# byronknoll/gmix

Measured on AMD Instinct MI355X. Metric: mixer bits/sec (synthetic 256-input mixer streams, forward+update), higher is better.
Workload: dtype f32; 1 GPU; configs[1]: synthetic 256-input 1-layer mixer (1 mixer, 2^16-row gate table), random logits, forward+update; n_inputs=256, mixers=1/0/0, streams_per_gpu=4096, total_bits=5465178112, parallelism=streams sharded over 1 GPU(s), no collective on the data path

## Files before the change

gmix_amd/csrc/gmx_capi.cpp:

```cpp
#include <hip/hip_runtime.h>
#include <math.h>
#include <stddef.h>
#include <stdio.h>
#include <stdlib.h>
#include <string.h>
#include <time.h>

#include <algorithm>
#include <atomic>
#include <map>
#include <new>
#include <string>
#include <vector>

#include "../../include/gmxmix.h"
#include "../../include/gmxmix_lstm_group.h"
#include "../../include/gmxmix_decoder.h"
#include "gmx_buildhash.h"
#include "gmx_internal.h"
#include "gmx_mailbox.h"
#include "gmx_batch_rows.h"
#include "gmx_ckpt.h"
#include "gmx_ckpt_stage.h"
#include "gmx_ind_ckpt.h"
// ... 291 lines not shown
    void *dst = up ? *col.dev : *col.host, *src = up ? *col.host : *col.dev;
    const GmxRowCopy r = gmx_row_copy(c->S, c->max_rows, n, col.row_bytes);
    if (r.height)
      HIPCHK(hipMemcpy2DAsync(dst, r.pitch, src, r.pitch, r.width, r.height, kind, st));
    else
      HIPCHK(hipMemcpyAsync(dst, src, r.bytes, kind, st));
  }
  for (const GmxBatchCol& col : c->cols) {
    if (col.dir != dir || !col.per_stream) continue;
    void *dst = up ? *col.dev : *col.host, *src = up ? *col.host : *col.dev;
    HIPCHK(hipMemcpyAsync(dst, src, gmx_col_host_bytes(col, c->S, c->max_rows), kind, st));
  }
  return up ? xfer_end_upload(c->x, main, st) : xfer_end_download(c->x, st);
}
static int batch_core_wait(GmxBatchCore* c) {
  if (!c || !c->bank) return GMX_ERR_INVALID;
  HIPCHK(hipSetDevice(c->bank->device));
  return xfer_wait(c->x);
}


static constexpr int kStageSlots = 4;
struct GmxCountList {
  uint64_t* dev[kStageSlots] = {};
  uint64_t* host[kStageSlots] = {};
  hipEvent_t done[kStageSlots] = {};
  bool busy[kStageSlots] = {};
  size_t cap = 0;
  unsigned seq = 0;
};
static void count_list_free(GmxCountList& c) {
  for (int k = 0; k < kStageSlots; ++k) {
    if (c.dev[k]) (void)hipFree(c.dev[k]);
    if (c.host[k]) (void)hipHostFree(c.host[k]);
    if (c.done[k]) (void)hipEventDestroy(c.done[k]);
  }
  c = GmxCountList();
}
static int count_list_stage(GmxCountList& c, const uint64_t* counts, int n, hipStream_t st, const uint64_t** dev_out) {
  const int k = (int)(c.seq++ % (unsigned)kStageSlots);
  if (c.busy[k]) {
    HIPCHK(hipEventSynchronize(c.done[k]));
    c.busy[k] = false;
  }
  if ((size_t)n > c.cap) {
    for (int j = 0; j < kStageSlots; ++j) {
      if (c.busy[j]) {
        HIPCHK(hipEventSynchronize(c.done[j]));
        c.busy[j] = false;
      }
      if (c.dev[j]) (void)hipFree(c.dev[j]);
      if (c.host[j]) (void)hipHostFree(c.host[j]);
      c.dev[j] = nullptr;
      c.host[j] = nullptr;
    }
    c.cap = 0;
    const size_t cap = (size_t)n + 64;
    for (int j = 0; j < kStageSlots; ++j) {
      HIPCHK(hipMalloc((void**)&c.dev[j], cap * sizeof(uint64_t)));
      HIPCHK(hipHostMalloc((void**)&c.host[j], cap * sizeof(uint64_t), hipHostMallocDefault));
      if (!c.done[j]) HIPCHK(hipEventCreateWithFlags(&c.done[j], hipEventDisableTiming));
    }
    c.cap = cap;
  }
  memcpy(c.host[k], counts, (size_t)n * sizeof(uint64_t));
  HIPCHK(hipMemcpyAsync(c.dev[k], c.host[k], (size_t)n * sizeof(uint64_t), hipMemcpyHostToDevice, st));
  *dev_out = c.dev[k];
  return GMX_OK;
}
static int count_list_used(GmxCountList& c, hipStream_t st) {
  const int k = (int)((c.seq - 1u) % (unsigned)kStageSlots);
  HIPCHK(hipEventRecord(c.done[k], st));
  c.busy[k] = true;
  return GMX_OK;
}

struct gmx_group {
  int device = 0;
  int S = 0;
  GmxTopoDev topo;
  GmxTopoDev* topo_dev = nullptr;
  uint8_t* banks = nullptr;
  float* latch_out = nullptr;
  hipStream_t stream = nullptr;
  hipEvent_t ev0 = nullptr, ev1 = nullptr;
  unsigned lds_bytes = 0;
  std::vector<uint64_t> steps;
  std::vector<uint8_t> fwd_done;
  struct DecaySlot {
    float* dev = nullptr;
    uint32_t* idx_dev = nullptr;
    float* host = nullptr;
    uint32_t* idx_host = nullptr;
    size_t cap = 0;
    size_t idx_cap = 0;
    hipEvent_t done = nullptr;
    hipEvent_t ready = nullptr;
    bool busy = false;
    uint64_t* st_dev = nullptr;
    uint64_t* st_host = nullptr;
    uint32_t* amb_dev = nullptr;
    uint32_t* amb_host = nullptr;
    float* patch_host = nullptr;
    size_t st_cap = 0;
  } decay[kStageSlots];
  GmxCountList counts;
  hipStream_t copy_stream = nullptr;
  hipStream_t up_stream = nullptr, down_stream = nullptr;
  unsigned run_seq = 0;
  hipEvent_t tm0 = nullptr, tm1 = nullptr;
  gmx_batch* one = nullptr;
  GmxBatchBank bb;
  std::vector<struct GmxSession*> sessions;
  std::vector<struct gmx_lockstep*> locksteps;
  bool banks_in_use_by_dead_kernel = false;
  bool use_sessions = true;
  bool mailbox_on_device = true;
  bool force_general = false;
  bool stock_exact = false;
  int stock_staged = -1;
  bool decay_on_host = false;
  bool stock_pairs = false;
  bool register_rows = false;
  int single_variant = 0;
  struct GmxCkptState* ckpt = nullptr;
};

struct gmx_batch : GmxBatchCore {
  gmx_group* g = nullptr;
  uint64_t& max_bits = max_rows;
  unsigned flags = 0;
  float* d_pred = nullptr;
  uint32_t* d_mask = nullptr;
  uint32_t* d_ctx = nullptr;
  uint8_t* d_bits = nullptr;
  float* d_p = nullptr;
  float* d_out = nullptr;
  float* d_last = nullptr;
  uint64_t* d_rng = nullptr;
  uint64_t* d_tcount = nullptr;
  float* d_pstate = nullptr;
  uint32_t* d_cstate = nullptr;
  float* h_pred = nullptr;
  uint32_t* h_mask = nullptr;
  uint32_t* h_ctx = nullptr;
  uint8_t* h_bits = nullptr;
  float* h_p = nullptr;
  float* h_out = nullptr;
  float* h_last = nullptr;
};

struct gmx_lockstep {
  gmx_group* g = nullptr;
  gmx_batch* b = nullptr;
  float* dec_host = nullptr;
  uint8_t* bits_host = nullptr;
  float* dec_dev = nullptr;
  uint32_t* idx_dev = nullptr;
  hipGraph_t g_predict = nullptr, g_learn = nullptr, g_step = nullptr;
  hipGraphExec_t x_predict = nullptr, x_learn = nullptr, x_step = nullptr;
  bool predicted = false;
  bool persistent = false, ps_running = false, ps_dead = false, ps_counted = false;
  hipStream_t ps_stream = nullptr;
  GmxLsDoor* door = nullptr;
  uint32_t* done = nullptr;
  uint32_t* blk_seen = nullptr;
// ... 125 lines not shown
      x.rs_off = x.w_off + (uint64_t)at * 4u;
      x.rs_pitch = x.stride * 4u;
    } else {
      x.rs_off = off;
      x.rs_pitch = 8u;
      off += (uint64_t)x.table_size * 8u;
      off = round_up64(off, 128);
    }
  }
  o->scal_off = off;
  off += (uint64_t)o->m * 24u;
  o->bank_bytes = round_up64(off, 256);
  uint32_t l = 0;
  o->lds_in0 = l;
  o->in0_sz = round_up((uint32_t)o->n_pad + (uint32_t)o->l0 + 4u, 4);
  l += 2 * o->in0_sz;
  o->lds_o1 = l;
  l += round_up((uint32_t)(o->l1 ? o->l1 : 1), 4);
  o->lds_skip = l;
  l += GMX_MAX_SKIP;
  o->lds_misc = l;
  l += 256;
  for (int grp = 0; grp < 2; ++grp) {
    const int lo = grp == 0 ? 0 : o->l0, hi = grp == 0 ? o->l0 : o->m;
    if (lo >= hi) continue;
    uint32_t dmax = 0;
    for (int j = lo; j < hi; ++j) dmax = std::max(dmax, o->mx[j].stride);
    const uint32_t D = dmax + 4;
    const uint32_t S = round_up((uint32_t)(hi - lo) * D, 64);
    for (int j = lo; j < hi; ++j) {
      o->mx[j].lds_off = l + (uint32_t)(j - lo) * D;
      o->mx[j].pitch = S;
    }
    l += 2 * S;
  }
  o->lds_total = l;
  if ((uint64_t)o->lds_total * 4u > 160u * 1024u) return GMX_ERR_INVALID;
  return GMX_OK;
}

static void batch_free(gmx_batch* b);
static int batch_alloc(gmx_batch** out, gmx_group* g, int S, uint64_t max_bits, unsigned flags);
static int batch_note_device_use(gmx_batch* b);

extern "C" int gmx_group_create(gmx_group** out, const gmx_topology* topo, int n_streams, int device) {
  if (!out || n_streams < 1) return GMX_ERR_INVALID;
  *out = nullptr;
  GmxTopoDev td;
  int rc = build_topology(topo, &td);
  if (rc) return rc;
  int ndev = 0;
  if (hipGetDeviceCount(&ndev) != hipSuccess || ndev <= 0) {
    (void)hipGetLastError();
    return GMX_ERR_NO_DEVICE;
  }
  if (device < 0 || device >= ndev) return GMX_ERR_INVALID;
  HIPCHK(hipSetDevice(device));
  gmx_group* g = new (std::nothrow) gmx_group();
  if (!g) return GMX_ERR_NOMEM;
  g->device = device;
  batch_bank_init(g->bb, g, device, &g->stream, &g->up_stream, &g->down_stream);
  g->S = n_streams;
  g->topo = td;
  g->lds_bytes = td.lds_total * 4u;
  g->steps.assign(n_streams, 0);
  g->fwd_done.assign(n_streams, 0);
#define GCHK(call)                                 \
  do {                                             \
    hipError_t e_ = (call);                        \
    if (e_ != hipSuccess) {                        \
      int r_ = hip_fail(e_, #call);                \
      gmx_group_destroy(g);                        \
      return e_ == hipErrorOutOfMemory ? GMX_ERR_NOMEM : r_; \
    }                                              \
  } while (0)
  GCHK(bank_stream_create(&g->stream, 0));
  GCHK(hipEventCreate(&g->ev0));
  GCHK(hipEventCreate(&g->ev1));
  GCHK(hipMalloc((void**)&g->topo_dev, sizeof(GmxTopoDev)));
  GCHK(hipMemcpy(g->topo_dev, &g->topo, sizeof(GmxTopoDev), hipMemcpyHostToDevice));
  GCHK(hipMalloc((void**)&g->banks, (size_t)n_streams * td.bank_bytes));
  GCHK(hipMalloc((void**)&g->latch_out, (size_t)n_streams * td.m * sizeof(float)));
  GCHK(hipMemsetAsync(g->latch_out, 0, (size_t)n_streams * td.m * sizeof(float), g->stream));
  if (g->lds_bytes > 48u * 1024u) GCHK(gmx_bank_kernel_set_lds(g->lds_bytes));
#undef GCHK
  rc = gmx_group_reset(g);
  if (rc) {
    gmx_group_destroy(g);
    return rc;
  }
  *out = g;
  return GMX_OK;
}

extern "C" void gmx_group_destroy(gmx_group* g) {
  if (!g) return;
  (void)hipSetDevice(g->device);
  sessions_free(g);
  if (g->stream) (void)hipStreamSynchronize(g->stream);
  if (g->one) {
    batch_free(g->one);
    g->one = nullptr;
  }
  for (gmx_lockstep* ls : g->locksteps) ls->g = nullptr;
  g->locksteps.clear();
  batch_bank_detach_all(g->bb);
  if (!g->banks_in_use_by_dead_kernel) {
    if (g->banks) (void)hipFree(g->banks);
    if (g->latch_out) (void)hipFree(g->latch_out);
    if (g->topo_dev) (void)hipFree(g->topo_dev);
  }
  for (auto& d : g->decay) {
    if (d.st_dev) (void)hipFree(d.st_dev);
    if (d.st_host) (void)hipHostFree(d.st_host);
    if (d.amb_dev) (void)hipFree(d.amb_dev);
    if (d.amb_host) (void)hipHostFree(d.amb_host);
    if (d.patch_host) (void)hipHostFree(d.patch_host);
    if (d.dev) (void)hipFree(d.dev);
    if (d.idx_dev) (void)hipFree(d.idx_dev);
    if (d.host) (void)hipHostFree(d.host);
    if (d.idx_host) (void)hipHostFree(d.idx_host);
    if (d.done) (void)hipEventDestroy(d.done);
    if (d.ready) (void)hipEventDestroy(d.ready);
  }
  count_list_free(g->counts);
  ckpt_free(g);
  if (g->copy_stream) (void)hipStreamDestroy(g->copy_stream);
  if (g->up_stream) {
    (void)hipStreamSynchronize(g->up_stream);
    (void)hipStreamDestroy(g->up_stream);
  }
  if (g->down_stream) {
    (void)hipStreamSynchronize(g->down_stream);
    (void)hipStreamDestroy(g->down_stream);
  }
  if (g->tm0) (void)hipEventDestroy(g->tm0);
  if (g->tm1) (void)hipEventDestroy(g->tm1);
  if (g->ev0) (void)hipEventDestroy(g->ev0);
  if (g->ev1) (void)hipEventDestroy(g->ev1);
  if (g->stream) (void)hipStreamDestroy(g->stream);
  delete g;
}

extern "C" int gmx_group_n_streams(const gmx_group* g) { return g ? g->S : GMX_ERR_INVALID; }
extern "C" int gmx_group_n_mixers(const gmx_group* g) { return g ? g->topo.m : GMX_ERR_INVALID; }
extern "C" int gmx_group_n_inputs(const gmx_group* g) { return g ? g->topo.n : GMX_ERR_INVALID; }
extern "C" uint64_t gmx_group_bank_bytes(const gmx_group* g) { return g ? g->topo.bank_bytes : 0; }

extern "C" int gmx_group_reset(gmx_group* g) {
  if (!g) return GMX_ERR_INVALID;
  HIPCHK(hipSetDevice(g->device));
  int rc = sessions_close(g, false);
  if (rc) return rc;
  HIPCHK(hipMemsetAsync(g->banks, 0, (size_t)g->S * g->topo.bank_bytes, g->stream));
  HIPCHK(gmx_launch_init_scal(g->banks, g->topo.bank_bytes, g->topo.scal_off, g->topo.m, g->S,
                              g->stream));
  HIPCHK(hipStreamSynchronize(g->stream));
  std::fill(g->steps.begin(), g->steps.end(), 0);
  std::fill(g->fwd_done.begin(), g->fwd_done.end(), 0);
  for (gmx_lockstep* ls : g->locksteps) ls->predicted = false;
  return GMX_OK;
}

extern "C" int gmx_group_sync(gmx_group* g) {
  if (!g) return GMX_ERR_INVALID;
  HIPCHK(hipSetDevice(g->device));
  int rc = sessions_close(g, true);
  if (rc) return rc;
  HIPCHK(hipStreamSynchronize(g->stream));
  return GMX_OK;
}

extern "C" int gmx_group_timer_start(gmx_group* g) {
  if (!g) return GMX_ERR_INVALID;
  HIPCHK(hipSetDevice(g->device));
  if (!g->tm0) {
    HIPCHK(hipEventCreate(&g->tm0));
    HIPCHK(hipEventCreate(&g->tm1));
  }
  HIPCHK(hipEventRecord(g->tm0, g->stream));
  return GMX_OK;
}

extern "C" int gmx_group_timer_stop(gmx_group* g, float* ms) {
  if (!g || !ms || !g->tm0) return GMX_ERR_INVALID;
  HIPCHK(hipSetDevice(g->device));
  HIPCHK(hipEventRecord(g->tm1, g->stream));
  HIPCHK(hipEventSynchronize(g->tm1));
  HIPCHK(hipEventElapsedTime(ms, g->tm0, g->tm1));
  return GMX_OK;
}

// ... 99 lines not shown
      }
      if (!e.done) {
        HIPCHK(hipEventCreateWithFlags(&e.done, hipEventDisableTiming));
        HIPCHK(hipEventCreateWithFlags(&e.ready, hipEventDisableTiming));
      }
    }
  }
  if (!g->copy_stream) HIPCHK(sibling_stream_create(&g->copy_stream, g->stream));
  bool on_device = false;
  if (learn && uniq.size() > 1 && uniq.size() * T >= kDecayDeviceMin && uniq.size() * T < (1ull << 32) &&
      !g->decay_on_host) {
    const int rcd = decay_table_on_device(g, d, uniq, T);
    if (rcd != GMX_OK && rcd != GMX_ERR_STATE) return rcd;
    on_device = rcd == GMX_OK;
  }
  if (!on_device) {
    for (auto& kv : uniq) {
      float* tab = d.host + (size_t)kv.second * T;
      if (learn)
        for (uint64_t t = 0; t < T; ++t) tab[t] = decay_base(kv.first + t);
      else
        for (uint64_t t = 0; t < T; ++t) tab[t] = 0.f;
    }
    HIPCHK(hipMemcpyAsync(d.dev, d.host, uniq.size() * T * sizeof(float), hipMemcpyHostToDevice, g->copy_stream));
  }
  memcpy(d.idx_host, idx.data(), ns * sizeof(uint32_t));
  HIPCHK(hipMemcpyAsync(d.idx_dev, d.idx_host, ns * sizeof(uint32_t), hipMemcpyHostToDevice, g->copy_stream));
  HIPCHK(hipEventRecord(d.ready, g->copy_stream));
  HIPCHK(hipStreamWaitEvent(g->stream, d.ready, 0));
  return GMX_OK;
}

static bool topo_register_rows_eligible(const GmxTopoDev& t) {
  return t.has_final && t.l0 >= 1 && t.l0 <= 24 && t.l1 >= 1 && t.l1 <= 8 && t.m == t.l0 + t.l1 + 1 &&
         t.n_skip == 1 && gmx_pair_kernel_half(t.n) != 0;
}

enum GmxKernelKind : int { GMX_K_SINGLE, GMX_K_WIDE, GMX_K_STOCK, GMX_K_BANK, GMX_K_PAIR };
static GmxKernelKind kernel_for(const gmx_group* g, unsigned mode) {
  if (g->register_rows && (mode & GMX_MODE_PREDICT) && !(mode & GMX_MODE_LATCH) && !g->force_general &&
      topo_register_rows_eligible(g->topo))
    return GMX_K_PAIR;
  const bool single = g->topo.m == 1 && g->topo.n <= 256 && (mode & GMX_MODE_PREDICT) &&
                      !(mode & GMX_MODE_LATCH) && !g->force_general;
  const bool stock = g->topo.n == 90 && g->topo.l0 == 24 && g->topo.l1 == 8 && g->topo.n_skip == 1 &&
                     g->topo.has_final && g->topo.mx[23].stride == 128 && !g->force_general;
  const bool wide = g->topo.l0 == 24 && g->topo.l1 == 8 && g->topo.n_skip == 1 && g->topo.has_final &&
                    ((g->topo.n == 256 && g->topo.mx[23].stride == 288) ||
                     (g->topo.n == 90 && g->topo.mx[23].stride == 128 && g->stock_pairs && !g->stock_exact)) &&
                    (mode & GMX_MODE_PREDICT) && !(mode & GMX_MODE_LATCH) && !g->force_general;
  return single ? GMX_K_SINGLE : wide ? GMX_K_WIDE : stock ? GMX_K_STOCK : GMX_K_BANK;
}

static int launch_run(gmx_group* g, gmx_batch* b, int s0, int rec0, int ns, uint64_t T,
                      unsigned mode, float* kernel_ms, const uint64_t* n_list = nullptr) {
  if (T == 0) return GMX_OK;
  for (gmx_lockstep* ls : g->locksteps) ls->predicted = false;
  gmx_group::DecaySlot* dec = nullptr;
  int rc = prepare_decay(g, s0, ns, T, (mode & GMX_MODE_LEARN) ? 1 : 0, &dec);
  if (rc) return rc;
  GmxRunArgs a;
  memset(&a, 0, sizeof a);
  a.banks = g->banks;
  a.pred = b->d_pred;
  a.mask = (b->flags & GMX_BATCH_MASK) ? b->d_mask : nullptr;
  a.ctx = b->d_ctx;
  a.bits = b->d_bits;
  a.decay = dec->dev;
  a.decay_idx = dec->idx_dev;
  a.p_out = b->d_p;
  a.out_all = (b->flags & GMX_BATCH_OUTPUTS) ? b->d_out : nullptr;
  a.out_last = (b->flags & GMX_BATCH_LAST_OUTPUTS) ? b->d_last : nullptr;
  a.latch_out = g->latch_out;
  a.rec_stride = b->max_bits;
  a.T = T;
  if (n_list) {
    int rcl = count_list_stage(g->counts, n_list, ns, g->stream, &a.T_list);
    if (rcl) return rcl;
  }
  a.mode = mode | (g->stock_exact ? GMX_MODE_EXACT : 0u);
  a.stream_base = s0;
  a.rec_base = rec0;
  a.n_streams = ns;
  {
    int rcx = xfer_before_run(b->x, g->stream);
    if (rcx) return rcx;
  }
  if (kernel_ms) HIPCHK(hipEventRecord(g->ev0, g->stream));
  const GmxKernelKind kind = kernel_for(g, mode);
  const bool single = kind == GMX_K_SINGLE, wide = kind == GMX_K_WIDE, stock = kind == GMX_K_STOCK;
  if (a.out_last && (single || wide)) return GMX_ERR_INVALID;
  if (kind == GMX_K_PAIR)
    HIPCHK(gmx_launch_pair_kernel(g->topo_dev, &a, ns, a.mask != nullptr, g->topo.n, g->topo.l0, g->topo.l1, g->stream));
  else if (single)
    HIPCHK(gmx_launch_single_kernel(g->topo_dev, &a, g->topo.n, g->single_variant, g->stream));
  else if (wide)
    HIPCHK(gmx_launch_wide_kernel(g->topo_dev, &a, ns, a.mask != nullptr, g->topo.n, g->stream));
  else if (stock)
    HIPCHK(gmx_launch_stock_kernel(g->topo_dev, &a, ns, GMX_STK_LDS_BYTES(g->topo.lds_misc),
                                   a.mask != nullptr, g->stock_staged, topo_tables_pow2(g->topo), g->stream));
  else
    HIPCHK(gmx_launch_bank_kernel(g->topo_dev, &a, ns, g->lds_bytes, a.mask != nullptr, g->topo.l0,
                                  g->topo.l1, g->topo.n_skip, g->topo.has_final,
                                  g->topo.mx[g->topo.l0 - 1].stride, g->stream));
  HIPCHK(hipEventRecord(dec->done, g->stream));
  dec->busy = true;
  if (n_list) {
    int rcl = count_list_used(g->counts, g->stream);
    if (rcl) return rcl;
  }
  {
    int rcn = batch_note_device_use(b);
    if (rcn) return rcn;
  }
  if (kernel_ms) {
    HIPCHK(hipEventRecord(g->ev1, g->stream));
    HIPCHK(hipEventSynchronize(g->ev1));
    HIPCHK(hipEventElapsedTime(kernel_ms, g->ev0, g->ev1));
  }
  if (mode & GMX_MODE_LEARN)
    for (int i = 0; i < ns; ++i) g->steps[s0 + i] += n_list ? n_list[i] : T;
  return GMX_OK;
}

static void batch_free(gmx_batch* b) {
  if (!b) return;
  batch_core_free(*b);
  delete b;
}

static int batch_alloc(gmx_batch** out, gmx_group* g, int S, uint64_t max_bits, unsigned flags) {
  if (!out || !g || max_bits == 0) return GMX_ERR_INVALID;
  *out = nullptr;
  gmx_batch* b = new (std::nothrow) gmx_batch();
  if (!b) return GMX_ERR_NOMEM;
  b->back = (void**)&b->g;
  b->flags = flags;
  gmx_mixer_batch_cols(b->cols, b, g->topo.n_pad, g->topo.m, g->topo.mask_words, flags);
  int rc = batch_core_alloc(*b, &g->bb, S, max_bits, false);
  if (rc) {
    batch_free(b);
    return rc;
  }
  *out = b;
  return GMX_OK;
}

extern "C" int gmx_batch_create(gmx_batch** out, gmx_group* g, uint64_t max_bits, unsigned flags) {
  if (!g) return GMX_ERR_INVALID;
  if (flags & GMX_BATCH_LAST_OUTPUTS) {
    const GmxKernelKind kind = kernel_for(g, GMX_MODE_PREDICT | GMX_MODE_LEARN);
    if ((kind == GMX_K_SINGLE || kind == GMX_K_WIDE) && !topo_register_rows_eligible(g->topo)) return GMX_ERR_INVALID;
  }
  int rc = batch_alloc(out, g, g->S, max_bits, flags);
  if (rc) return rc;
  return xfer_streams_ready(g->stream, &g->up_stream, &g->down_stream);
}

extern "C" void gmx_batch_destroy(gmx_batch* b) { batch_free(b); }
extern "C" int gmx_batch_n_pad(const gmx_batch* b) { return (b && b->g) ? b->g->topo.n_pad : GMX_ERR_INVALID; }
extern "C" int gmx_batch_mask_words(const gmx_batch* b) { return (b && b->g) ? b->g->topo.mask_words : GMX_ERR_INVALID; }
extern "C" uint64_t gmx_batch_max_bits(const gmx_batch* b) { return b ? b->max_bits : 0; }

extern "C" float* gmx_batch_predictions(gmx_batch* b) { return b ? (float*)batch_core_host(*b, &b->h_pred) : nullptr; }
extern "C" uint32_t* gmx_batch_active_mask(gmx_batch* b) {
  return b ? (uint32_t*)batch_core_host(*b, &b->h_mask) : nullptr;
// ... 937 lines not shown
```

gmix_amd/csrc/gmx_internal.h:

```cpp
#ifndef GMX_INTERNAL_H_
#define GMX_INTERNAL_H_

#include <stdint.h>

#define GMX_MAX_MIXERS 64
#define GMX_MAX_SKIP 8
#define GMX_MAX_INPUTS 2048

#define GMX_MODE_PREDICT 1u
#define GMX_MODE_LEARN 2u
#define GMX_MODE_LATCH 4u
#define GMX_MODE_EXACT 8u

struct GmxMixerDev {
  uint32_t table_size;
  uint32_t weight_size;
  uint32_t stride;
  uint32_t lds_off;
  uint32_t pitch;
  int32_t layer;
  int32_t out_index;
  float lr;
  uint64_t w_off;
  uint64_t rs_off;
  uint32_t rs_pitch;
  uint32_t rs_folded;
};

#define GMX_RS_PTR(bank, mx, row) \
  ((uint64_t*)((uint8_t*)(bank) + (mx).rs_off + (uint64_t)(row) * (mx).rs_pitch))

struct GmxTopoDev {
  int32_t n, n_pad, n_skip, m, l0, l1, has_final, mask_words;
  int32_t skip_idx[GMX_MAX_SKIP];
  uint32_t lds_in0;
  uint32_t in0_sz;
  uint32_t lds_o1;
  uint32_t lds_skip;
  uint32_t lds_misc;
  uint32_t lds_total;
  uint64_t scal_off;
  uint64_t bank_bytes;
  GmxMixerDev mx[GMX_MAX_MIXERS];
};

struct GmxRunArgs {
  uint8_t* banks;
  const float* pred;
  const uint32_t* mask;
  const uint32_t* ctx;
  const uint8_t* bits;
  const float* decay;
  const uint32_t* decay_idx;
  float* p_out;
  float* out_all;
  float* out_last;
  float* latch_out;
  uint64_t rec_stride;
  uint64_t T;
  const uint64_t* T_list;
  uint32_t mode;
  int32_t stream_base;
  int32_t rec_base;
  int32_t n_streams;
};

#define GMX_STK_LDS_BYTES(lds_misc) (((lds_misc) + 256u) * 4u + 2u * 33u * 528u)

#define GMX_MB_FORWARD 1u
#define GMX_MB_LEARN0 2u
#define GMX_MB_LEARN1 3u
#define GMX_MB_STOP 4u
#define GMX_MB_LEARN0_FWD 5u
#define GMX_MB_LEARN1_FWD 6u
#define GMX_MB_STOP_KEEP 7u
#define GMX_MB_CMD_MASK 7u
#define GMX_MB_SLOT_SHIFT 3
#define GMX_MB_SEQ_SHIFT 4
#define GMX_MB_RUNNING 0u
#define GMX_MB_EXIT_IDLE 1u
#define GMX_MB_EXIT_STOP 2u
struct GmxMbPayload {
  uint32_t dec_bits;
  uint32_t pad0[3];
  uint32_t mask[4];
  uint32_t ctx[36];
  uint32_t pad1[4];
  float pred[96];
};
struct GmxMbCmd {
  uint32_t cmd_seq;
  uint32_t pad0[15];
  GmxMbPayload slot[2];
};
struct GmxMbReply {
  uint32_t done_seq;
  uint32_t state;
  float p;
  uint32_t pad[13];
  float outs[48];
};

struct GmxLsDoor {
  uint32_t cmd_seq;
  uint32_t pad[15];
};
struct GmxLsArgs {
  uint8_t* banks;
  GmxLsDoor* door;
  uint32_t* done;
  const float* pred;
  const uint32_t* mask;
  const uint32_t* ctx;
  const uint8_t* bits;
  const float* dec;
  float* p;
  float* outs;
  uint32_t* blk_seen;
  uint32_t* blk_replay;
  uint32_t* relay;
  float* live;
  uint64_t idle_ticks;
  int32_t n_streams, exact;
};
#define GMX_LS_LIVE_FLOATS 160

struct GmxStkStepArgs {
  uint8_t* banks;
  const uint8_t* what;
  const uint8_t* bits;
  const float* dec;
  const float* pred_old;
  const uint32_t* mask_old;
  const uint32_t* ctx_old;
  const float* pred_new;
  const uint32_t* mask_new;
  const uint32_t* ctx_new;
  float* p_out;
  float* out_all;
  float* latch;
  const uint32_t* seq;
  uint32_t* stamp;
  int32_t n_streams, exact;
};

#define GMX_STEP_UP_MAX 12
struct GmxStepUpload {
  const uint8_t* src;
// ... 182 lines not shown
```

gmix_amd/csrc/gmx_single.hip:

```cpp
#include <hip/hip_runtime.h>
#include <stdint.h>

#include "gmx_internal.h"
#include "gmx_math.h"

typedef float gmx_f4 __attribute__((ext_vector_type(4)));

template <int OFF>
__device__ __forceinline__ void gmx_ld16(gmx_f4& d, const float* p) {
  asm volatile("global_load_dwordx4 %0, %1, off offset:%2 nt" : "=v"(d) : "v"(p), "n"(OFF) : "memory");
}
__device__ __forceinline__ void gmx_ld8(uint64_t& d, const uint64_t* p) {
  asm volatile("global_load_dwordx2 %0, %1, off" : "=v"(d) : "v"(p) : "memory");
}
__device__ __forceinline__ void gmx_ld4(uint32_t& d, const void* p) {
  asm volatile("global_load_dword %0, %1, off" : "=v"(d) : "v"(p) : "memory");
}
__device__ __forceinline__ void gmx_ld1(uint32_t& d, const uint8_t* p) {
  asm volatile("global_load_ubyte %0, %1, off" : "=v"(d) : "v"(p) : "memory");
}
template <int OFF>
__device__ __forceinline__ void gmx_st16(float* p, const gmx_f4& v) {
  asm volatile("global_store_dwordx4 %0, %1, off offset:%2 nt" : : "v"(p), "v"(v), "n"(OFF) : "memory");
}
__device__ __forceinline__ void gmx_st8(uint64_t* p, uint64_t v) {
  asm volatile("global_store_dwordx2 %0, %1, off" : : "v"(p), "v"(v) : "memory");
}
__device__ __forceinline__ void gmx_st4(float* p, float v) {
  asm volatile("global_store_dword %0, %1, off" : : "v"(p), "v"(v) : "memory");
}

template <int K>
struct GmxSlot {
  gmx_f4 w[K];
  gmx_f4 x[K];
  uint32_t mk[K];
  uint64_t rs;
  uint32_t row;
  uint32_t bit;
  uint32_t dec;
};

template <int N>
__device__ __forceinline__ void gmx_wait_slot(GmxSlot<1>& a) {
  asm volatile("s_waitcnt vmcnt(%c5)"
               : "+v"(a.w[0]), "+v"(a.x[0]), "+v"(a.rs), "+v"(a.bit), "+v"(a.dec)
               : "n"(N));
}
template <int N>
__device__ __forceinline__ void gmx_wait_slot(GmxSlot<2>& a) {
  asm volatile("s_waitcnt vmcnt(%c7)"
               : "+v"(a.w[0]), "+v"(a.w[1]), "+v"(a.x[0]), "+v"(a.x[1]), "+v"(a.rs), "+v"(a.bit),
                 "+v"(a.dec)
               : "n"(N));
}
template <int N>
__device__ __forceinline__ void gmx_wait_slot(GmxSlot<4>& a) {
  asm volatile("s_waitcnt vmcnt(%c11)"
               : "+v"(a.w[0]), "+v"(a.w[1]), "+v"(a.w[2]), "+v"(a.w[3]), "+v"(a.x[0]), "+v"(a.x[1]),
                 "+v"(a.x[2]), "+v"(a.x[3]), "+v"(a.rs), "+v"(a.bit), "+v"(a.dec)
               : "n"(N));
}
template <int K>
__device__ __forceinline__ void gmx_pin_mask(GmxSlot<K>& a) {
  if (K == 1) asm volatile("" : "+v"(a.mk[0]));
  if (K == 2) asm volatile("" : "+v"(a.mk[0]), "+v"(a.mk[1 % K]));
  if (K == 4) asm volatile("" : "+v"(a.mk[0]), "+v"(a.mk[1 % K]), "+v"(a.mk[2 % K]), "+v"(a.mk[3 % K]));
}
__device__ __forceinline__ void gmx_pin(uint64_t& rs, uint32_t& bit, uint32_t& dec, uint32_t& cq) {
  asm volatile("" : "+v"(rs), "+v"(bit), "+v"(dec), "+v"(cq));
}

template <int LPS>
__device__ __forceinline__ float gmx_handoff(float acc, int i, bool first_pass, int lane) {
  const int a = __float_as_int(acc);
  if (LPS == 64)
    return __int_as_float(__builtin_amdgcn_update_dpp(0, a, 0x13C, 0xf, 0xf, false));
  if (LPS == 16)
    return __int_as_float(__builtin_amdgcn_update_dpp(0, a, 0x121, 0xf, 0xf, false));
  if (i == 16)
    return __int_as_float(__builtin_amdgcn_update_dpp(a, a, 0x142, 0xa, 0xf, false));
  if (i == 0 && !first_pass)
    return __shfl(acc, (lane & 32) | 31);
  return __int_as_float(__builtin_amdgcn_update_dpp(0, a, 0x121, 0xf, 0xf, false));
}

template <int K, int LPS>
__device__ __forceinline__ float gmx_chain_piece(const GmxSlot<K>& c, int q, float acc, int lane) {
  const float px = c.x[q].x * c.w[q].x, py = c.x[q].y * c.w[q].y;
  const float pz = c.x[q].z * c.w[q].z, pw = c.x[q].w * c.w[q].w;
#pragma unroll
  for (int i = 0; i < LPS; ++i) {
    acc = gmx_handoff<LPS>(acc, i, q == 0, lane) + px;
    acc = acc + py;
    acc = acc + pz;
    acc = acc + pw;
  }
  return acc;
}
template <int K, int LPS>
__device__ __forceinline__ float gmx_chain(const GmxSlot<K>& c, int lane) {
  float acc = 0.f;
#pragma unroll
  for (int q = 0; q < K; ++q) acc = gmx_chain_piece<K, LPS>(c, q, acc, lane);
  return acc;
}

template <int LPS, int K, int NSLOT, bool FULL, bool WANT_OUT, bool LEARN, bool HAS_MASK>
__global__ void __launch_bounds__(64)
gmx_single_kernel(const GmxTopoDev* __restrict__ tp, const GmxRunArgs a) {
  constexpr int G = 64 / LPS;
  constexpr int CH = 4 * LPS;
  constexpr int VM_PER_BIT = 1 + (WANT_OUT ? 1 : 0) + (LEARN ? K + 1 : 0) + 2 * K + 3 + (HAS_MASK ? K : 0) + 1;
  constexpr int VM_WAIT = 1 + (NSLOT - 2) * VM_PER_BIT;
  static_assert(VM_WAIT <= 63, "vmcnt is a 6-bit counter");
  static_assert(CH * 4 * (K - 1) < 4096, "immediate offset of global_load is 12 bits");
  const int lane = threadIdx.x;
  const int g = lane / LPS, l = lane % LPS;
  const int li = (int)blockIdx.x * G + g;
  __shared__ uint64_t s_tab[32];
  if (lane < 32) s_tab[lane] = gmx_exp2f_tab[lane];
  if (li >= a.n_streams) return;
  const int rec = a.rec_base + li;
  const int s = a.stream_base + li;
  const uint64_t T = a.T;
  if (T == 0) return;

  const int N = tp->n, NPAD = tp->n_pad;
  const uint32_t stride = FULL ? (uint32_t)(CH * K) : tp->mx[0].stride;
  const uint32_t table = tp->mx[0].table_size;
  const float lr = tp->mx[0].lr;
  uint8_t* const bank = a.banks + (uint64_t)s * tp->bank_bytes;
  float* const wtab = (float*)(bank + tp->mx[0].w_off);
  uint64_t* const rstab = (uint64_t*)(bank + tp->mx[0].rs_off);
  uint64_t* const scal = (uint64_t*)(bank + tp->scal_off);

  const uint64_t RS = a.rec_stride;
  const uint32_t xstride = FULL ? (uint32_t)(CH * K) : (uint32_t)NPAD;
  const float* const pred_s = a.pred + (uint64_t)rec * RS * xstride;
  const uint32_t* const ctx_s = a.ctx + (uint64_t)rec * RS;
  const uint8_t* const bits_s = a.bits + (uint64_t)rec * RS;
  const float* const dec_s = a.decay + (uint64_t)a.decay_idx[li] * T;
  const int MW = tp->mask_words;
  const uint32_t* const mask_s = HAS_MASK ? a.mask + (uint64_t)rec * RS * MW : nullptr;
  float* const p_s = a.p_out + (uint64_t)rec * RS;
  float* const oa_s = WANT_OUT ? a.out_all + (uint64_t)rec * RS : nullptr;

  uint64_t steps = scal[0], max_steps = scal[1], seen_cnt = scal[2];

  GmxSlot<K> sl[NSLOT];
  uint32_t ctxq[NSLOT];

  auto issue = [&](GmxSlot<K>& d, uint32_t ctx, uint64_t tb) {
    const uint64_t tt = tb < T ? tb : T - 1;
    d.row = ctx % table;
    const float* wr = wtab + (uint64_t)d.row * stride + 4 * l;
    const float* xr = pred_s + tt * (uint64_t)xstride + 4 * l;
    if (FULL) {
      gmx_ld16<0>(d.w[0], wr);
      if (K > 1) gmx_ld16<CH * 4>(d.w[1 % K], wr);
      if (K > 2) gmx_ld16<CH * 8>(d.w[2 % K], wr);
      if (K > 3) gmx_ld16<CH * 12>(d.w[3 % K], wr);
      gmx_ld16<0>(d.x[0], xr);
      if (K > 1) gmx_ld16<CH * 4>(d.x[1 % K], xr);
      if (K > 2) gmx_ld16<CH * 8>(d.x[2 % K], xr);
      if (K > 3) gmx_ld16<CH * 12>(d.x[3 % K], xr);
    } else {
#pragma unroll
      for (int k = 0; k < K; ++k) {
        const int e = CH * k + 4 * l;
        gmx_ld16<0>(d.w[k], (uint32_t)e < stride ? wr + CH * k : wr - 4 * l);
      }
#pragma unroll
      for (int k = 0; k < K; ++k) {
        const int e = CH * k + 4 * l;
        gmx_ld16<0>(d.x[k], e < NPAD ? xr + CH * k : xr - 4 * l);
      }
    }
    if (HAS_MASK) {
#pragma unroll
      for (int k = 0; k < K; ++k) {
        const int e = CH * k + 4 * l;
        gmx_ld4(d.mk[k], mask_s + tt * (uint64_t)MW + (e < NPAD ? (e >> 5) : 0));
      }
    }
    gmx_ld8(d.rs, rstab + d.row);
    gmx_ld1(d.bit, bits_s + tt);
    gmx_ld4(d.dec, dec_s + tt);
  };
  auto mask_inputs = [&](GmxSlot<K>& d) {
    if (!HAS_MASK) return;
#pragma unroll
    for (int k = 0; k < K; ++k) {
      const uint32_t b = d.mk[k] >> ((uint32_t)(CH * k + 4 * l) & 31u);
      d.x[k].x = (b & 1u) ? d.x[k].x : 0.f;
      d.x[k].y = (b & 2u) ? d.x[k].y : 0.f;
      d.x[k].z = (b & 4u) ? d.x[k].z : 0.f;
      d.x[k].w = (b & 8u) ? d.x[k].w : 0.f;
    }
  };
  auto trim = [&](GmxSlot<K>& d) {
    if (FULL) return;
#pragma unroll
    for (int k = 0; k < K; ++k) {
      const int e = CH * k + 4 * l;
      const bool wok = (uint32_t)e < stride;
      d.w[k].x = wok ? d.w[k].x : 0.f;
      d.w[k].y = wok ? d.w[k].y : 0.f;
      d.w[k].z = wok ? d.w[k].z : 0.f;
      d.w[k].w = wok ? d.w[k].w : 0.f;
      d.x[k].x = (e + 0 < N) ? d.x[k].x : 0.f;
      d.x[k].y = (e + 1 < N) ? d.x[k].y : 0.f;
      d.x[k].z = (e + 2 < N) ? d.x[k].z : 0.f;
      d.x[k].w = (e + 3 < N) ? d.x[k].w : 0.f;
    }
  };

#pragma unroll
  for (int k = 0; k < NSLOT; ++k) {
    const uint64_t tb = (uint64_t)k < T ? (uint64_t)k : T - 1;
    ctxq[k] = ctx_s[tb];
  }
#pragma unroll
  for (int k = 0; k < NSLOT; ++k) {
    issue(sl[k], ctxq[k], (uint64_t)k);
    const uint64_t tb = (uint64_t)(k + NSLOT) < T ? (uint64_t)(k + NSLOT) : T - 1;
    gmx_ld4(ctxq[k], ctx_s + tb);
  }
#pragma unroll
  for (int k = 0; k < NSLOT; ++k) {
    gmx_wait_slot<0>(sl[k]);
    if (HAS_MASK) gmx_pin_mask(sl[k]);
    gmx_pin(sl[k].rs, sl[k].bit, sl[k].dec, ctxq[k]);
  }
  trim(sl[0]);
  mask_inputs(sl[0]);
  float acc_cur = gmx_chain<K, LPS>(sl[0], lane);

  for (uint64_t t0 = 0; t0 < T; t0 += NSLOT) {
#pragma unroll
    for (int k = 0; k < NSLOT; ++k) {
      const uint64_t t = t0 + k;
      if (t >= T) break;
      GmxSlot<K>& c = sl[k];
      GmxSlot<K>& nx = sl[(k + 1) % NSLOT];
      gmx_wait_slot<VM_WAIT>(nx);
      if (HAS_MASK) gmx_pin_mask(nx);
      gmx_pin(c.rs, c.bit, c.dec, ctxq[k]);
      trim(nx);
      mask_inputs(nx);
      float acc_nxt = gmx_chain_piece<K, LPS>(nx, 0, 0.f, lane);
      float out = __shfl(acc_cur, lane | (LPS - 1));
      const bool seen = c.rs != 0;
      out = seen ? out : 0.f;
      const float pl = gmx_logistic_tab(out, s_tab);
      const float prob = gmx_clamp_prob(pl);
      gmx_st4(p_s + t, prob);
      if (WANT_OUT) gmx_st4(oa_s + t, out);
      if (K > 1) acc_nxt = gmx_chain_piece<K, LPS>(nx, 1 % K, acc_nxt, lane);
      if (!LEARN) {
        if (K > 2) acc_nxt = gmx_chain_piece<K, LPS>(nx, 2 % K, acc_nxt, lane);
        if (K > 3) acc_nxt = gmx_chain_piece<K, LPS>(nx, 3 % K, acc_nxt, lane);
      } else {
        const double dd = (double)__uint_as_float(c.dec) * (1.5 - ((double)c.rs) / (double)max_steps);
        const float decay = (float)dd;
        const float upd = decay * lr * (pl - (float)c.bit);
        const uint64_t rs_new = c.rs + 1;
        ++steps;
        max_steps = rs_new > max_steps ? rs_new : max_steps;
        seen_cnt += (c.rs == 0) ? 1u : 0u;
        const float sc = ((rs_new & 1023u) == 0) ? (1.0f - 3.0e-6f) : 1.0f;
        if (K > 2) acc_nxt = gmx_chain_piece<K, LPS>(nx, 2 % K, acc_nxt, lane);
#pragma unroll
        for (int q = 0; q < K; ++q) {
          c.w[q].x = (c.w[q].x - upd * c.x[q].x) * sc;
          c.w[q].y = (c.w[q].y - upd * c.x[q].y) * sc;
          c.w[q].z = (c.w[q].z - upd * c.x[q].z) * sc;
          c.w[q].w = (c.w[q].w - upd * c.x[q].w) * sc;
        }
        float* wr = wtab + (uint64_t)c.row * stride + 4 * l;
        if (FULL) {
          gmx_st16<0>(wr, c.w[0]);
          if (K > 1) gmx_st16<CH * 4>(wr, c.w[1 % K]);
          if (K > 2) gmx_st16<CH * 8>(wr, c.w[2 % K]);
          if (K > 3) gmx_st16<CH * 12>(wr, c.w[3 % K]);
        } else {
#pragma unroll
          for (int q = 0; q < K; ++q)
            if ((uint32_t)(CH * q + 4 * l) < stride) gmx_st16<0>(wr + CH * q, c.w[q]);
        }
        gmx_st8(rstab + c.row, rs_new);
        if (K > 3) acc_nxt = gmx_chain_piece<K, LPS>(nx, 3 % K, acc_nxt, lane);
        bool hit[NSLOT];
        bool any_hit = false;
#pragma unroll
        for (int j = 1; j < NSLOT; ++j) {
          hit[j] = sl[(k + j) % NSLOT].row == c.row && (t + j) < T;
          any_hit |= hit[j];
        }
        if (__any(any_hit)) {
#pragma unroll
          for (int j = 2; j < NSLOT; ++j) gmx_wait_slot<0>(sl[(k + j) % NSLOT]);
#pragma unroll
          for (int j = 1; j < NSLOT; ++j) {
            GmxSlot<K>& o = sl[(k + j) % NSLOT];
            if (hit[j]) {
#pragma unroll
              for (int q = 0; q < K; ++q) o.w[q] = c.w[q];
              o.rs = rs_new;
            }
          }
          if (__any(hit[1])) acc_nxt = gmx_chain<K, LPS>(nx, lane);
        }
      }
      issue(c, ctxq[k], t + NSLOT);
      {
        const uint64_t tn = t + 2 * NSLOT;
        gmx_ld4(ctxq[k], ctx_s + (tn < T ? tn : T - 1));
      }
      acc_cur = acc_nxt;
    }
  }
  asm volatile("s_waitcnt vmcnt(0)" ::: "memory");
  if (LEARN) {
    scal[0] = steps;
    scal[1] = max_steps;
    scal[2] = seen_cnt;
  }
}

template <int LPS, int K, int NSLOT, bool FULL, bool HAS_MASK>
static hipError_t launch_kfm(const GmxTopoDev* tp_dev, const GmxRunArgs& a, hipStream_t stream) {
  constexpr int G = 64 / LPS;
  const dim3 grid((a.n_streams + G - 1) / G), block(64);
  const bool learn = (a.mode & GMX_MODE_LEARN) != 0;
  if (a.out_all) {
    if (learn)
      hipLaunchKernelGGL((gmx_single_kernel<LPS, K, NSLOT, FULL, true, true, HAS_MASK>), grid, block, 0, stream, tp_dev, a);
    else
      hipLaunchKernelGGL((gmx_single_kernel<LPS, K, NSLOT, FULL, true, false, HAS_MASK>), grid, block, 0, stream, tp_dev, a);
  } else {
    if (learn)
      hipLaunchKernelGGL((gmx_single_kernel<LPS, K, NSLOT, FULL, false, true, HAS_MASK>), grid, block, 0, stream, tp_dev, a);
    else
      hipLaunchKernelGGL((gmx_single_kernel<LPS, K, NSLOT, FULL, false, false, HAS_MASK>), grid, block, 0, stream, tp_dev, a);
  }
  return hipGetLastError();
}
template <int LPS, int K, int NSLOT, bool FULL>
static hipError_t launch_kf(const GmxTopoDev* tp_dev, const GmxRunArgs& a, hipStream_t stream) {
  constexpr int VM_M = 1 + 1 + (K + 1) + 2 * K + 3 + K + 1;
  constexpr int NS_M = (1 + (NSLOT - 2) * VM_M <= 63) ? NSLOT : NSLOT - 1;
  return a.mask ? launch_kfm<LPS, K, NS_M, FULL, true>(tp_dev, a, stream)
                : launch_kfm<LPS, K, NSLOT, FULL, false>(tp_dev, a, stream);
}

template <int LPS, int K, int NSLOT>
static hipError_t launch_k(const GmxTopoDev* tp_dev, const GmxRunArgs& a, bool full,
                           hipStream_t stream) {
  return full ? launch_kf<LPS, K, NSLOT, true>(tp_dev, a, stream)
              : launch_kf<LPS, K, NSLOT, false>(tp_dev, a, stream);
}

extern "C" hipError_t gmx_launch_single_kernel(const GmxTopoDev* tp_dev, const GmxRunArgs* args,
                                               int n_inputs, int variant, hipStream_t stream) {
  (void)hipGetLastError();
  const GmxRunArgs& a = *args;
  if (n_inputs <= 64) return launch_k<16, 1, 4>(tp_dev, a, n_inputs == 64, stream);
  if (n_inputs <= 128) {
    if (variant == 16) return launch_k<16, 2, 4>(tp_dev, a, n_inputs == 128, stream);
    return launch_k<32, 1, 6>(tp_dev, a, n_inputs == 128, stream);
  }
  const bool full = n_inputs == 256;
  if (variant == 165) return launch_k<16, 4, 5>(tp_dev, a, full, stream);
  if (variant == 325) return launch_k<32, 2, 5>(tp_dev, a, full, stream);
  if (variant == 64) return launch_k<64, 1, 6>(tp_dev, a, full, stream);
  if (variant == 32) return launch_k<32, 2, 4>(tp_dev, a, full, stream);
  return launch_k<16, 4, 4>(tp_dev, a, full, stream);
}
```

Measured before the change: 1.839 billion bits/s.

## Prefetch row state to redirect weight loads for unseen rows to a zero pad

Adds a second-level context prefetch so the kernel can load each row's step counter one pipeline stage ahead. Rows that have never been updated (state zero) get their weight loads redirected to a small shared zero-filled buffer instead of the large gate table. This is meant to cut scattered DRAM traffic when many rows are still fresh. In exchange it adds an extra load and registers per slot (AGPRs for K=4) and a stall-and-reload path when a skipped row becomes stale. It also lowers the slot count for some learn configurations to stay within the vmcnt limit.

```diff
diff --git a/gmix_amd/csrc/gmx_capi.cpp b/gmix_amd/csrc/gmx_capi.cpp
--- a/gmix_amd/csrc/gmx_capi.cpp
+++ b/gmix_amd/csrc/gmx_capi.cpp
@@ -397,6 +397,7 @@
   GmxTopoDev* topo_dev = nullptr;
   uint8_t* banks = nullptr;
   float* latch_out = nullptr;
+  float* zero_pad = nullptr;
   hipStream_t stream = nullptr;
   hipEvent_t ev0 = nullptr, ev1 = nullptr;
   unsigned lds_bytes = 0;
@@ -688,6 +689,8 @@
   GCHK(hipMalloc((void**)&g->banks, (size_t)n_streams * td.bank_bytes));
   GCHK(hipMalloc((void**)&g->latch_out, (size_t)n_streams * td.m * sizeof(float)));
   GCHK(hipMemsetAsync(g->latch_out, 0, (size_t)n_streams * td.m * sizeof(float), g->stream));
+  GCHK(hipMalloc((void**)&g->zero_pad, (size_t)GMX_ZPAD_SLICES * GMX_ZPAD_SLICE_FLOATS * sizeof(float)));
+  GCHK(hipMemsetAsync(g->zero_pad, 0, (size_t)GMX_ZPAD_SLICES * GMX_ZPAD_SLICE_FLOATS * sizeof(float), g->stream));
   if (g->lds_bytes > 48u * 1024u) GCHK(gmx_bank_kernel_set_lds(g->lds_bytes));
 #undef GCHK
   rc = gmx_group_reset(g);
@@ -714,6 +717,7 @@
   if (!g->banks_in_use_by_dead_kernel) {
     if (g->banks) (void)hipFree(g->banks);
     if (g->latch_out) (void)hipFree(g->latch_out);
+    if (g->zero_pad) (void)hipFree(g->zero_pad);
     if (g->topo_dev) (void)hipFree(g->topo_dev);
   }
   for (auto& d : g->decay) {
@@ -979,6 +983,7 @@
   a.stream_base = s0;
   a.rec_base = rec0;
   a.n_streams = ns;
+  a.zero_pad = g->zero_pad;
   {
     int rcx = xfer_before_run(b->x, g->stream);
     if (rcx) return rcx;
diff --git a/gmix_amd/csrc/gmx_internal.h b/gmix_amd/csrc/gmx_internal.h
--- a/gmix_amd/csrc/gmx_internal.h
+++ b/gmix_amd/csrc/gmx_internal.h
@@ -63,7 +63,10 @@
   int32_t stream_base;
   int32_t rec_base;
   int32_t n_streams;
-};
+  const float* zero_pad;
+};
+#define GMX_ZPAD_SLICE_FLOATS 256
+#define GMX_ZPAD_SLICES 64
 
 #define GMX_STK_LDS_BYTES(lds_misc) (((lds_misc) + 256u) * 4u + 2u * 33u * 528u)
 
diff --git a/gmix_amd/csrc/gmx_single.hip b/gmix_amd/csrc/gmx_single.hip
--- a/gmix_amd/csrc/gmx_single.hip
+++ b/gmix_amd/csrc/gmx_single.hip
@@ -37,6 +37,7 @@
   uint32_t mk[K];
   uint64_t rs;
   uint32_t row;
+  uint32_t skipped;
   uint32_t bit;
   uint32_t dec;
 };
@@ -69,6 +70,32 @@
 }
 __device__ __forceinline__ void gmx_pin(uint64_t& rs, uint32_t& bit, uint32_t& dec, uint32_t& cq) {
   asm volatile("" : "+v"(rs), "+v"(bit), "+v"(dec), "+v"(cq));
+}
+template <bool ACC>
+__device__ __forceinline__ void gmx_ldq(uint32_t& d, const void* p) {
+  if (ACC)
+    asm volatile("global_load_dword %0, %1, off" : "=a"(d) : "v"(p) : "memory");
+  else
+    asm volatile("global_load_dword %0, %1, off" : "=v"(d) : "v"(p) : "memory");
+}
+template <bool ACC>
+__device__ __forceinline__ void gmx_pinq(uint32_t& pk, uint32_t& cq) {
+  if (ACC)
+    asm volatile("" : "+a"(pk), "+v"(cq));
+  else
+    asm volatile("" : "+v"(pk), "+v"(cq));
+}
+__device__ __forceinline__ uint32_t gmx_take_unseen(const uint32_t& pk) {
+  uint32_t u = pk == 0 ? 1u : 0u;
+  asm volatile("" : "+v"(u));
+  return u;
+}
+__device__ __forceinline__ void gmx_wait_row(gmx_f4 (&w)[1]) { asm volatile("s_waitcnt vmcnt(0)" : "+v"(w[0])); }
+__device__ __forceinline__ void gmx_wait_row(gmx_f4 (&w)[2]) {
+  asm volatile("s_waitcnt vmcnt(0)" : "+v"(w[0]), "+v"(w[1]));
+}
+__device__ __forceinline__ void gmx_wait_row(gmx_f4 (&w)[4]) {
+  asm volatile("s_waitcnt vmcnt(0)" : "+v"(w[0]), "+v"(w[1]), "+v"(w[2]), "+v"(w[3]));
 }
 
 template <int LPS>
@@ -111,9 +138,10 @@
 gmx_single_kernel(const GmxTopoDev* __restrict__ tp, const GmxRunArgs a) {
   constexpr int G = 64 / LPS;
   constexpr int CH = 4 * LPS;
-  constexpr int VM_PER_BIT = 1 + (WANT_OUT ? 1 : 0) + (LEARN ? K + 1 : 0) + 2 * K + 3 + (HAS_MASK ? K : 0) + 1;
-  constexpr int VM_WAIT = 1 + (NSLOT - 2) * VM_PER_BIT;
+  constexpr int VM_PER_BIT = 1 + (WANT_OUT ? 1 : 0) + (LEARN ? K + 1 : 0) + 1 + 2 * K + 3 + (HAS_MASK ? K : 0) + 2;
+  constexpr int VM_WAIT = 2 + (NSLOT - 2) * VM_PER_BIT;
   static_assert(VM_WAIT <= 63, "vmcnt is a 6-bit counter");
+  constexpr bool QACC = K == 4;
   static_assert(CH * 4 * (K - 1) < 4096, "immediate offset of global_load is 12 bits");
   const int lane = threadIdx.x;
   const int g = lane / LPS, l = lane % LPS;
@@ -134,6 +162,7 @@
   float* const wtab = (float*)(bank + tp->mx[0].w_off);
   uint64_t* const rstab = (uint64_t*)(bank + tp->mx[0].rs_off);
   uint64_t* const scal = (uint64_t*)(bank + tp->scal_off);
+  const float* const zpad = a.zero_pad + (blockIdx.x % GMX_ZPAD_SLICES) * GMX_ZPAD_SLICE_FLOATS + 4 * l;
 
   const uint64_t RS = a.rec_stride;
   const uint32_t xstride = FULL ? (uint32_t)(CH * K) : (uint32_t)NPAD;
@@ -150,27 +179,36 @@
 
   GmxSlot<K> sl[NSLOT];
   uint32_t ctxq[NSLOT];
-
-  auto issue = [&](GmxSlot<K>& d, uint32_t ctx, uint64_t tb) {
+  uint32_t ctxq2[NSLOT];
+  uint32_t pkq[NSLOT];
+
+  auto load_row = [&](gmx_f4 (&w)[K], uint32_t row, bool to_pad) {
+    const float* wr = to_pad ? zpad : wtab + (uint64_t)row * stride + 4 * l;
+    if (FULL) {
+      gmx_ld16<0>(w[0], wr);
+      if (K > 1) gmx_ld16<CH * 4>(w[1 % K], wr);
+      if (K > 2) gmx_ld16<CH * 8>(w[2 % K], wr);
+      if (K > 3) gmx_ld16<CH * 12>(w[3 % K], wr);
+    } else {
+#pragma unroll
+      for (int k = 0; k < K; ++k) {
+        const int e = CH * k + 4 * l;
+        gmx_ld16<0>(w[k], (uint32_t)e < stride ? wr + CH * k : wr - 4 * l);
+      }
+    }
+  };
+  auto issue = [&](GmxSlot<K>& d, uint32_t ctx, uint64_t tb, uint32_t unseen) {
     const uint64_t tt = tb < T ? tb : T - 1;
     d.row = ctx % table;
-    const float* wr = wtab + (uint64_t)d.row * stride + 4 * l;
+    d.skipped = unseen;
     const float* xr = pred_s + tt * (uint64_t)xstride + 4 * l;
+    load_row(d.w, d.row, unseen != 0);
     if (FULL) {
-      gmx_ld16<0>(d.w[0], wr);
-      if (K > 1) gmx_ld16<CH * 4>(d.w[1 % K], wr);
-      if (K > 2) gmx_ld16<CH * 8>(d.w[2 % K], wr);
-      if (K > 3) gmx_ld16<CH * 12>(d.w[3 % K], wr);
       gmx_ld16<0>(d.x[0], xr);
       if (K > 1) gmx_ld16<CH * 4>(d.x[1 % K], xr);
       if (K > 2) gmx_ld16<CH * 8>(d.x[2 % K], xr);
       if (K > 3) gmx_ld16<CH * 12>(d.x[3 % K], xr);
     } else {
-#pragma unroll
-      for (int k = 0; k < K; ++k) {
-        const int e = CH * k + 4 * l;
-        gmx_ld16<0>(d.w[k], (uint32_t)e < stride ? wr + CH * k : wr - 4 * l);
-      }
 #pragma unroll
       for (int k = 0; k < K; ++k) {
         const int e = CH * k + 4 * l;
@@ -216,23 +254,34 @@
     }
   };
 
-#pragma unroll
-  for (int k = 0; k < NSLOT; ++k) {
-    const uint64_t tb = (uint64_t)k < T ? (uint64_t)k : T - 1;
-    ctxq[k] = ctx_s[tb];
-  }
-#pragma unroll
-  for (int k = 0; k < NSLOT; ++k) {
-    issue(sl[k], ctxq[k], (uint64_t)k);
-    const uint64_t tb = (uint64_t)(k + NSLOT) < T ? (uint64_t)(k + NSLOT) : T - 1;
-    gmx_ld4(ctxq[k], ctx_s + tb);
+  {
+    uint32_t c0[NSLOT];
+    uint64_t p0[NSLOT];
+#pragma unroll
+    for (int k = 0; k < NSLOT; ++k) {
+      const uint64_t tb = (uint64_t)k < T ? (uint64_t)k : T - 1;
+      const uint64_t tn = (uint64_t)(k + NSLOT) < T ? (uint64_t)(k + NSLOT) : T - 1;
+      c0[k] = ctx_s[tb];
+      ctxq[k] = ctx_s[tn];
+    }
+#pragma unroll
+    for (int k = 0; k < NSLOT; ++k) p0[k] = rstab[c0[k] % table];
+#pragma unroll
+    for (int k = 0; k < NSLOT; ++k) {
+      gmx_ldq<QACC>(pkq[k], rstab + ctxq[k] % table);
+      issue(sl[k], c0[k], (uint64_t)k, p0[k] == 0 ? 1u : 0u);
+      const uint64_t tb = (uint64_t)(k + 2 * NSLOT) < T ? (uint64_t)(k + 2 * NSLOT) : T - 1;
+      gmx_ld4(ctxq2[k], ctx_s + tb);
+    }
   }
 #pragma unroll
   for (int k = 0; k < NSLOT; ++k) {
     gmx_wait_slot<0>(sl[k]);
     if (HAS_MASK) gmx_pin_mask(sl[k]);
     gmx_pin(sl[k].rs, sl[k].bit, sl[k].dec, ctxq[k]);
-  }
+    gmx_pinq<QACC>(pkq[k], ctxq2[k]);
+  }
+  asm volatile("" : "+v"(steps), "+v"(max_steps), "+v"(seen_cnt));
   trim(sl[0]);
   mask_inputs(sl[0]);
   float acc_cur = gmx_chain<K, LPS>(sl[0], lane);
@@ -247,6 +296,18 @@
       gmx_wait_slot<VM_WAIT>(nx);
       if (HAS_MASK) gmx_pin_mask(nx);
       gmx_pin(c.rs, c.bit, c.dec, ctxq[k]);
+      gmx_pinq<QACC>(pkq[k], ctxq2[k]);
+      if (LEARN) {
+        const bool stale = nx.skipped != 0 && nx.rs != 0 && (t + 1) < T;
+        if (__any(stale)) {
+#pragma unroll
+          for (int j = 2; j < NSLOT; ++j) gmx_wait_slot<0>(sl[(k + j) % NSLOT]);
+          asm volatile("s_waitcnt vmcnt(0)" ::: "memory");
+          nx.skipped = stale ? 0u : nx.skipped;
+          load_row(nx.w, nx.row, nx.skipped != 0);
+          gmx_wait_row(nx.w);
+        }
+      }
       trim(nx);
       mask_inputs(nx);
       float acc_nxt = gmx_chain_piece<K, LPS>(nx, 0, 0.f, lane);
@@ -308,15 +369,19 @@
 #pragma unroll
               for (int q = 0; q < K; ++q) o.w[q] = c.w[q];
               o.rs = rs_new;
+              o.skipped = 0;
             }
           }
           if (__any(hit[1])) acc_nxt = gmx_chain<K, LPS>(nx, lane);
         }
       }
-      issue(c, ctxq[k], t + NSLOT);
       {
-        const uint64_t tn = t + 2 * NSLOT;
+        const uint32_t unseen = gmx_take_unseen(pkq[k]);
+        gmx_ldq<QACC>(pkq[k], rstab + ctxq2[k] % table);
+        issue(c, ctxq[k], t + NSLOT, unseen);
+        const uint64_t tn = t + 2 * NSLOT, tp = t + 3 * NSLOT;
         gmx_ld4(ctxq[k], ctx_s + (tn < T ? tn : T - 1));
+        gmx_ld4(ctxq2[k], ctx_s + (tp < T ? tp : T - 1));
       }
       acc_cur = acc_nxt;
     }
@@ -334,14 +399,16 @@
   constexpr int G = 64 / LPS;
   const dim3 grid((a.n_streams + G - 1) / G), block(64);
   const bool learn = (a.mode & GMX_MODE_LEARN) != 0;
+  constexpr int NS_L = (K * NSLOT > 16) ? NSLOT - 1 : NSLOT;
+  constexpr int NS_LF = FULL ? NSLOT : NS_L;
   if (a.out_all) {
     if (learn)
-      hipLaunchKernelGGL((gmx_single_kernel<LPS, K, NSLOT, FULL, true, true, HAS_MASK>), grid, block, 0, stream, tp_dev, a);
+      hipLaunchKernelGGL((gmx_single_kernel<LPS, K, NS_L, FULL, true, true, HAS_MASK>), grid, block, 0, stream, tp_dev, a);
     else
       hipLaunchKernelGGL((gmx_single_kernel<LPS, K, NSLOT, FULL, true, false, HAS_MASK>), grid, block, 0, stream, tp_dev, a);
   } else {
     if (learn)
-      hipLaunchKernelGGL((gmx_single_kernel<LPS, K, NSLOT, FULL, false, true, HAS_MASK>), grid, block, 0, stream, tp_dev, a);
+      hipLaunchKernelGGL((gmx_single_kernel<LPS, K, NS_LF, FULL, false, true, HAS_MASK>), grid, block, 0, stream, tp_dev, a);
     else
       hipLaunchKernelGGL((gmx_single_kernel<LPS, K, NSLOT, FULL, false, false, HAS_MASK>), grid, block, 0, stream, tp_dev, a);
   }
@@ -349,8 +416,8 @@
 }
 template <int LPS, int K, int NSLOT, bool FULL>
 static hipError_t launch_kf(const GmxTopoDev* tp_dev, const GmxRunArgs& a, hipStream_t stream) {
-  constexpr int VM_M = 1 + 1 + (K + 1) + 2 * K + 3 + K + 1;
-  constexpr int NS_M = (1 + (NSLOT - 2) * VM_M <= 63) ? NSLOT : NSLOT - 1;
+  constexpr int VM_M = 1 + 1 + (K + 1) + 1 + 2 * K + 3 + K + 2;
+  constexpr int NS_M = (2 + (NSLOT - 2) * VM_M <= 63) ? NSLOT : NSLOT - 1;
   return a.mask ? launch_kfm<LPS, K, NS_M, FULL, true>(tp_dev, a, stream)
                 : launch_kfm<LPS, K, NSLOT, FULL, false>(tp_dev, a, stream);
 }
```

Result: no change. 1.842 billion bits/s (median of 5 runs) (+0.1%).
